# DreamOneX/yet-another-bpe

Measured on AMD Instinct MI355X. Metric: merges_per_sec, higher is better.
Workload: dtype u16

## Files before the change

include/yabpe.h:

```cpp
#ifndef YABPE_H
#define YABPE_H

#include <stddef.h>
#include <stdint.h>

#ifdef __cplusplus
extern "C" {
#endif

#define YABPE_ABI_VERSION 2

enum {
    YABPE_OK = 0,
    YABPE_E_INVALID = -1,
    YABPE_E_NODEVICE = -2,
    YABPE_E_HIP = -3,
    YABPE_E_CAPACITY = -4,
    YABPE_E_INTERNAL = -5,
    YABPE_E_COMM = -6,
    YABPE_E_UTF8 = -7
};

#define YABPE_LOAD_DEDUP 0x1u

// ... 44 lines not shown
    uint64_t table_entries;
    uint64_t retiles, table_rebuilds;
    double load_ms;
    double train_ms;
    double apply_ms_sampled;
    uint64_t apply_launches_sampled;
    uint64_t apply_algo_bytes_sampled;
    uint64_t apply_actual_bytes_sampled;
    uint64_t algo_bytes_total;
    double scan_ms_sampled;
    uint64_t scan_launches_sampled;
    uint64_t scan_algo_bytes_sampled;
    uint64_t scan_actual_bytes_sampled;
    uint64_t scan_skip_launches;
    uint64_t scan_skip_tiles_read;
    uint64_t cand_rebuilds;
    uint64_t cand_rescans;
    uint64_t fused_launches;
    double dense_ms_sampled;
    uint64_t dense_launches_sampled;
    uint64_t dense_algo_bytes_sampled;
    uint64_t dense_actual_bytes_sampled;
    double sparse_ms;
    uint64_t sparse_merges;
    double tail_ms;
    uint64_t tail_merges;
    uint64_t exchanges, exchange_bytes, exchange_cap_records, exchange_growths, exchange_max_records;
    uint64_t sparse_launches;
    uint64_t tail_launches;
    double exchange_ms_sampled;
    uint64_t exchanges_sampled;
    uint64_t exchange_p2p;
    uint64_t dense_launches, dense_merges;
} yabpe_stats_t;
int yabpe_stats(yabpe_ctx *ctx, yabpe_stats_t *out);
int yabpe_iter_log(yabpe_ctx *ctx, uint64_t *out_sites, uint64_t *out_live_slots, uint32_t cap, uint32_t *out_n);

int yabpe_event_log(yabpe_ctx *ctx, uint32_t *out_iter, float *out_us, float *out_scan_us, uint32_t cap, uint32_t *out_n);

typedef struct yabpe_latency_t {
    double launch_gap_us;
    double load_trip_us;
    double coherent_trip_us;
    double atomic_trip_us;
} yabpe_latency_t;
int yabpe_latency_probe(yabpe_ctx *ctx, yabpe_latency_t *out);

int yabpe_verify_table(yabpe_ctx *ctx, uint64_t *out_mismatches);
int yabpe_stream_checksum(yabpe_ctx *ctx, uint64_t *out_sum, uint64_t *out_words, uint64_t *out_tokens);

int yabpe_synth_generate(yabpe_ctx *ctx, uint64_t target_bytes, uint32_t n_types, uint64_t seed,
                         const uint8_t *alphabet, uint32_t alphabet_len, int space_prefix,
                         uint8_t **out_dev_bytes, uint64_t **out_dev_off, uint64_t *out_n_words, uint64_t *out_n_bytes);
int yabpe_synth_generate_lex(yabpe_ctx *ctx, uint64_t target_bytes, uint32_t n_types, uint64_t seed,
                             const uint8_t *lex_bytes, const uint64_t *lex_off,
                             uint8_t **out_dev_bytes, uint64_t **out_dev_off, uint64_t *out_n_pieces, uint64_t *out_n_bytes);
int yabpe_synth_free(yabpe_ctx *ctx);
int yabpe_memcpy_d2h(yabpe_ctx *ctx, void *dst_host, const void *src_dev, uint64_t n);
int yabpe_memcpy_h2d(yabpe_ctx *ctx, void *dst_dev, const void *src_host, uint64_t n);

int yabpe_pretokenize(yabpe_ctx *ctx, const uint8_t *text, uint64_t n_bytes, const uint64_t *chunk_off, uint32_t n_chunks,
                      const uint8_t *special_bytes, const uint32_t *special_off, uint32_t n_special,
                      const uint8_t **out_dev_text, uint64_t **out_dev_word_off, uint64_t *out_n_words, int64_t *out_bad_pos);
int yabpe_pretokenize_free(yabpe_ctx *ctx);

int yabpe_pool_add(yabpe_ctx *ctx, const uint8_t *bytes, const uint64_t *word_off, const uint64_t *word_freq, uint64_t n_words);
// ... 109 lines not shown
```

yet-another-bpe_amd/csrc/yabpe.hip:

```cpp
#include <hip/hip_runtime.h>
#include <dlfcn.h>
#include <rccl/rccl.h>

#include <algorithm>
#include <cstdarg>
#include <cstddef>
#include <cstdio>
#include <cstring>
#include <map>
#include <mutex>
#include <string>
#include <vector>

#include "../../include/yabpe.h"
#include "yabpe_kernels.h"
#include "yabpe_aux_kernels.h"
#include "yabpe_devmem.h"
#include "yabpe_pretok_kernels.h"
#include "yabpe_encode_kernels.h"
#include "yabpe_dropout_kernels.h"
#include "yabpe_decode_kernels.h"
#include "yabpe_layout_kernels.h"
#include "yabpe_replay_kernels.h"
#include "yabpe_pool_kernels.h"
// ... 19 lines not shown
        tried = true;
        std::vector<std::string> names;
        Dl_info info;
        if (dladdr((void *)&hipGetDeviceCount, &info) && info.dli_fname) {
            std::string dir(info.dli_fname);
            const size_t slash = dir.rfind('/');
            if (slash != std::string::npos) {
                dir.resize(slash);
                names.push_back(dir + "/librccl.so.1");
                names.push_back(dir + "/librccl.so");
            }
        }
        names.push_back("librccl.so.1");
        names.push_back("librccl.so");
        for (const auto &name : names) {
            r.h = dlopen(name.c_str(), RTLD_NOW | RTLD_LOCAL);
            if (r.h) break;
        }
        if (r.h) {
            r.GetUniqueId = (decltype(r.GetUniqueId))dlsym(r.h, "ncclGetUniqueId");
            r.CommInitRank = (decltype(r.CommInitRank))dlsym(r.h, "ncclCommInitRank");
            r.AllGather = (decltype(r.AllGather))dlsym(r.h, "ncclAllGather");
            r.AllReduce = (decltype(r.AllReduce))dlsym(r.h, "ncclAllReduce");
            r.CommDestroy = (decltype(r.CommDestroy))dlsym(r.h, "ncclCommDestroy");
            r.GetErrorString = (decltype(r.GetErrorString))dlsym(r.h, "ncclGetErrorString");
            if (!r.GetUniqueId || !r.CommInitRank || !r.AllGather || !r.AllReduce || !r.CommDestroy) r.h = nullptr;
        }
    }
    return r.h ? &r : nullptr;
}

constexpr uint32_t MAX_APPLY_BLOCKS = 8192;
constexpr uint32_t MAX_LISTS = 2048;
thread_local std::string g_create_error;

struct EventPair {
    hipEvent_t e0, e1, e2;
    uint32_t iter_rel;
    bool split;
};

}

struct yabpe_ctx {
    int device = 0;
    int n_cu = 256;
    int apply_occ = 4;
    hipStream_t stream = nullptr;
    std::string err;
    std::map<std::string, int64_t> opt;

    bool have_vocab = false;
    uint32_t base_tokens = 0;
    TokTable tt{};
    bool have_words = false;
    bool weighted = false;
    uint64_t n_words = 0, n_words_input = 0, tokens_initial = 0;
    uint32_t n_tiles = 0;
    uint16_t *tiles = nullptr, *tiles_alt = nullptr;
    uint32_t tiles_cap = 0, tiles_alt_cap = 0;
    uint32_t *tile_len = nullptr, *tile_len_alt = nullptr;
    uint32_t *tile_wbase = nullptr, *tile_wbase_alt = nullptr;
    uint32_t *wfreq = nullptr;
    uint32_t n_long = 0;
    uint16_t *long_tok = nullptr;
    unsigned long long *long_sig = nullptr;
// ... 31 lines not shown
    unsigned long long *enc_spans = nullptr;
    yabpe_encode_stats_t enc_stats{};
    unsigned long long enc_sums[4] = {0, 0, 0, 0};
    bool enc_done = false;
    hipEvent_t enc_ev[8] = {};
    bool have_dec_model = false;
    uint2 *dec_ent = nullptr;
    uint8_t *dec_pool = nullptr;
    uint32_t dec_n = 0;
    uint8_t *dec_text = nullptr;
    unsigned long long *dec_doc = nullptr;
    yabpe_decode_stats_t dec_stats{};
    hipEvent_t dec_ev[7] = {};
    uint32_t *lay_buf[3] = {};
    yabpe_layout_stats_t lay_stats{};
    hipEvent_t lay_ev[4] = {};
    yabpe_resume_stats_t resume_stats{};
    bool have_pool = false;
    PoolView wpool{};
    uint64_t wpool_arena_cap = 0, wpool_n = 0, wpool_bytes = 0;
    yabpe_pool_stats_t wpool_stats{};
    hipEvent_t wpool_ev[4] = {};
    unsigned long long *scratch64 = nullptr;
    unsigned long long *blk_stats = nullptr;
    uint32_t blk_used = 0;
    bool split_mode = false;
    uint32_t kmax_now = 1;
    uint32_t rec_n_live = 0;
    std::vector<float> ev_scan_us;
    unsigned long long *sig = nullptr;
    uint32_t sig_stride = 0;
    unsigned long long *blk_read = nullptr;
    uint64_t scan_skip_launches = 0;
    bool sig_valid = false;
    uint32_t sig_built_at = 0;
    uint64_t sig_tokens_at_build = 0;
    uint64_t sig_builds = 0;
    CandState *cand_state = nullptr;
    uint32_t cand_built_at = 0;
    unsigned long long cand_best_at_build = 0;
    uint32_t *sel_ticket = nullptr;
    unsigned long long *cand = nullptr;
    bool use_cand = false;
    uint64_t cand_rebuilds = 0, cand_rescans = 0;
    double cand_margin = 0.2;
    uint32_t cand_n_at_build = 0;
    bool pending = false;
    uint64_t fused_launches = 0;
    int rank = 0, n_ranks = 1;
    bool multi = false;
    ncclComm_t comm = nullptr;
    yabpe_allgather_fn ag_fn = nullptr;
    void *ag_user = nullptr;
    unsigned long long *xsmall = nullptr;
    uint8_t *xsend = nullptr, *xrecv = nullptr;
    uint64_t exchange_growths = 0;
    uint64_t exchange_max_records = 0;
    uint32_t xcap = 0;
    uint64_t xstride = 0;
    uint32_t xeff = 0;
    uint64_t xeff_sum = 0;
    uint32_t xseen[4] = {0, 0, 0, 0};
    uint64_t exchanges = 0;
    bool p2p = false;
    uint8_t *p2p_area = nullptr;
    std::vector<uint8_t *> p2p_peer;
// ... 1024 lines not shown
    c->stats.retiles = 0;
    c->stats.train_ms = 0;
    c->stats.apply_ms_sampled = 0;
    c->stats.apply_launches_sampled = 0;
    c->stats.apply_algo_bytes_sampled = 0;
    c->stats.apply_actual_bytes_sampled = 0;
    c->stats.dense_ms_sampled = 0;
    c->stats.dense_launches_sampled = 0;
    c->stats.dense_launches = 0;
    c->stats.dense_merges = 0;
    c->stats.dense_algo_bytes_sampled = 0;
    c->stats.dense_actual_bytes_sampled = 0;
    c->stats.sparse_ms = 0;
    c->stats.sparse_merges = 0;
    c->stats.sparse_launches = 0;
    c->stats.tail_ms = 0;
    c->stats.tail_merges = 0;
    c->stats.tail_launches = 0;
    c->stats.exchange_ms_sampled = 0;
    c->stats.exchanges_sampled = 0;
    c->stats.scan_ms_sampled = 0;
    c->stats.scan_launches_sampled = 0;
    c->stats.scan_algo_bytes_sampled = 0;
    c->stats.scan_actual_bytes_sampled = 0;
    c->scan_skip_launches = 0;
    c->cand_rebuilds = c->cand_rescans = 0;
    c->fused_launches = 0;
    c->exchanges = 0;
    c->xeff = c->xcap;
    c->xseen[0] = c->xseen[1] = c->xseen[2] = c->xseen[3] = 0;
    c->xeff_sum = 0;
    c->exchange_growths = 0;
    c->exchange_max_records = 0;
    if (c->blk_read) HIPCHK(c, hipMemsetAsync(c->blk_read, 0, MAX_LISTS * 8, c->stream));
    c->stats.algo_bytes_total = 0;
    c->have_words = true;
    return YABPE_OK;
}

int yabpe_load_words(yabpe_ctx *c, const uint8_t *bytes, const uint64_t *word_off, const uint64_t *word_freq,
                     uint64_t n_words, uint32_t flags) {
    if (!c) return YABPE_E_INVALID;
    return load_words_impl(c, bytes, word_off, word_freq, n_words, flags, nullptr);
}

int yabpe_load_words_resumed(yabpe_ctx *c, const uint8_t *bytes, const uint64_t *word_off, const uint64_t *word_freq, uint64_t n_words,
                             uint32_t flags, const uint32_t *merge_left, const uint32_t *merge_right, const uint32_t *merge_merged,
                             uint32_t n_merges) {
    if (!c) return YABPE_E_INVALID;
    HIPCHK(c, hipSetDevice(c->device));
    if (!c->have_vocab) return fail(c, YABPE_E_INVALID, "call yabpe_set_vocab first (with all of the model's tokens)");
    if (n_merges == 0) return load_words_impl(c, bytes, word_off, word_freq, n_words, flags, nullptr);
    if (!word_freq && !(flags & YABPE_LOAD_DEDUP))
        return fail(c, YABPE_E_INVALID, "a resumed load needs the pooled layout: pass word_freq or YABPE_LOAD_DEDUP");
    if (c->multi) return fail(c, YABPE_E_INVALID, "a resumed load on several GPUs is not supported");
    if (!merge_left || !merge_right || !merge_merged) return fail(c, YABPE_E_INVALID, "merge triples are NULL");
    TRY(state_pull(c));
    const uint32_t n_tokens = c->st_host->n_tokens;
    std::vector<uint32_t> len(n_tokens);
    HIPCHK(c, hipMemcpy(len.data(), c->tt.len, (size_t)n_tokens * 4, hipMemcpyDeviceToHost));
    for (uint32_t i = 0; i < n_merges; ++i) {
        const uint32_t l = merge_left[i], r = merge_right[i], m = merge_merged[i];
        if (l >= n_tokens || r >= n_tokens || m >= n_tokens)
            return fail(c, YABPE_E_INVALID, "merge %u names token id %u, the vocabulary has %u", i, std::max(l, std::max(r, m)), n_tokens);
        if (len[m] != len[l] + len[r])
            return fail(c, YABPE_E_INVALID, "merge %u: token %u has %u bytes, its operands %u + %u", i, m, len[m], len[l], len[r]);
    }
// ... 81 lines not shown
            F.ticket = c->sel_ticket;
            F.sel = select_params(c, rec_base, 0u, std::max(c->blk_used, grid_now));
        }
        return F;
    };
    if (c->n_tiles) {
        ApplyParams P{c->tiles, c->tile_len, c->tile_wbase, c->wfreq, c->n_tiles, out_table, c->st, c->blk_stats,
                      c->split_mode ? c->sig : nullptr, c->sig_stride, (uint32_t)AGG_N - 1u, 1u};
        if (!c->split_mode) {
            const FuseParams F = fuse_params(apply_grid);
            const uint32_t rr_blocks = rank_rides ? rank_blocks : 0u;
            c->blk_used = std::max(c->blk_used, apply_grid);
            if (c->weighted)
                hipLaunchKernelGGL(k_apply<true>, dim3(apply_grid + rr_blocks + long_blocks), dim3(BLOCK), 0, c->stream, P, apply_grid, R, F, LW, apply_grid + rr_blocks);
            else if (optv(c, "hist", 1) && tokens_upper <= (uint32_t)HIST_V)
                hipLaunchKernelGGL((k_apply<false, true>), dim3(apply_grid + rr_blocks + long_blocks), dim3(BLOCK), 0, c->stream, P, apply_grid, R, F, LW, apply_grid + rr_blocks);
            else
                hipLaunchKernelGGL(k_apply<false>, dim3(apply_grid + rr_blocks + long_blocks), dim3(BLOCK), 0, c->stream, P, apply_grid, R, F, LW, apply_grid + rr_blocks);
            if (ev) HIPCHK(c, hipEventRecord(ev->e1, c->stream));
        } else {
            if (!sparse) return fail(c, YABPE_E_INTERNAL, "sparse form without signatures");
            int64_t wpb_opt = optv(c, "full_wpb", 0);
            if (wpb_opt <= 0)
                wpb_opt = (c->st_host->best_count <= (unsigned long long)optv(c, "wide_sites_per_cu", 20) * c->n_cu && (c->n_tiles + 2047u) / 2048u <= c->n_cu) ? 16 : 8;
            const uint32_t nw = wpb_opt >= 16 ? 16u : 8u;
            const uint32_t nt = nw * 64u;
            const uint32_t target = (uint32_t)std::max<int64_t>(1, optv(c, "full_skip_blocks", (int64_t)c->n_cu * (16 / nw)));
            const uint32_t ktm = (uint32_t)scan_kt_max((int)nw);
            const uint32_t chunk = std::min<uint32_t>(nt * ktm, std::max<uint32_t>(64u, (uint32_t)(((uint64_t)(c->n_tiles + target - 1) / target + 63u) / 64u * 64u)));
            const uint32_t kt = (chunk + nt - 1) / nt;
            const uint32_t n_chunks = (c->n_tiles + chunk - 1) / chunk;
            const uint32_t scan_grid = std::max(1u, std::min<uint32_t>(std::min<uint32_t>(n_chunks, target), MAX_LISTS));
            if (!c->blk_read) {
                TRY(dmalloc(c, &c->blk_read, MAX_LISTS));
                HIPCHK(c, hipMemsetAsync(c->blk_read, 0, MAX_LISTS * 8, c->stream));
            }
            if (optv(c, "agg_small", 1) && !c->weighted && c->st_host->best_count * 4 < 48ull * std::max<uint32_t>(1u, c->n_cu * 3))
                P.agg_mask = (uint32_t)(c->kmax_now > 2 ? AGG_N : nw >= 16 ? AGG_N / 2 : AGG_N / 4) - 1u;
            const uint32_t rr_blocks = rank_rides ? rank_blocks : 0u;
            ScanSkipParams SQ{P, c->blk_read, scan_grid, kt, chunk, R, fuse_params(scan_grid), LW, scan_grid + rr_blocks};
            c->blk_used = std::max(c->blk_used, scan_grid);
            const uint32_t grid = scan_grid + rr_blocks + long_blocks;
#define YB_LAUNCH_SPARSE(NW_)                                                                                        \
    do {                                                                                                             \
        if (c->weighted)                                                                                             \
            hipLaunchKernelGGL((k_scan_skip<true, NW_>), dim3(grid), dim3(NW_ * 64), 0, c->stream, c->st, SQ);      \
        else                                                                                                         \
            hipLaunchKernelGGL((k_scan_skip<false, NW_>), dim3(grid), dim3(NW_ * 64), 0, c->stream, c->st, SQ);     \
    } while (0)
            if (nw == 16) YB_LAUNCH_SPARSE(16);
            else YB_LAUNCH_SPARSE(8);
#undef YB_LAUNCH_SPARSE
            c->scan_skip_launches++;
            if (ev) HIPCHK(c, hipEventRecord(ev->e1, c->stream));
        }
    } else if (ev) {
        HIPCHK(c, hipEventRecord(ev->e1, c->stream));
    }
    if (ev) HIPCHK(c, hipEventRecord(ev->e2, c->stream));
    if (!fuse_kernel && c->n_long) hipLaunchKernelGGL(k_apply_long, dim3(cdiv64(c->n_long, long_group)), dim3(BLOCK), 0, c->stream, LW);
    if (c->multi) {
        const uint64_t xbytes = 16 + (uint64_t)c->xeff * sizeof(DeltaRec);
        const uint8_t *recv = c->xrecv;
        uint64_t rstride = xbytes;
        if (c->p2p) {
            XchgParams X{};
            X.send = c->xsend;
            for (int r = 0; r < c->n_ranks; ++r) X.peer[r] = c->p2p_peer[r];
            X.flags_off = c->p2p_flags_off;
            X.half_bytes = c->p2p_half;
            X.stride = c->p2p_stride;
            X.seq = ++c->p2p_seq;
            X.rank = (uint32_t)c->rank;
// ... 458 lines not shown
    uint32_t off = 0, len = 0;
    HIPCHK(c, hipMemcpy(&off, c->tt.off + id, 4, hipMemcpyDeviceToHost));
    HIPCHK(c, hipMemcpy(&len, c->tt.len + id, 4, hipMemcpyDeviceToHost));
    *out_len = len;
    if (out && cap >= len && len) HIPCHK(c, hipMemcpy(out, c->tt.pool + off, len, hipMemcpyDeviceToHost));
    return YABPE_OK;
}

int yabpe_stats(yabpe_ctx *c, yabpe_stats_t *out) {
    if (!c || !out) return YABPE_E_INVALID;
    HIPCHK(c, hipSetDevice(c->device));
    TRY(state_pull(c));
    c->stats.n_words = c->n_words;
    c->stats.n_words_input = c->n_words_input;
    c->stats.n_long_words = c->n_long;
    c->stats.tokens_initial = c->tokens_initial;
    c->stats.tokens_now = c->st_host->tokens_now;
    c->stats.merges_done = c->st_host->iter;
    c->stats.n_tiles = c->n_tiles;
    c->stats.live_slots = c->st_host->live_slots;
    c->stats.table_capacity = c->table_cap;
    c->stats.table_entries = c->st_host->table_entries;
    c->stats.cand_rebuilds = c->cand_rebuilds;
    c->stats.cand_rescans = c->cand_rescans;
    c->stats.fused_launches = c->fused_launches;
    c->stats.exchanges = c->exchanges;
    c->stats.exchange_bytes = (c->multi && c->exchanges) ? (16 + (c->xeff_sum / c->exchanges) * sizeof(DeltaRec)) * (uint64_t)c->n_ranks : 0;
    c->stats.exchange_cap_records = c->xcap;
    c->stats.exchange_p2p = c->p2p ? 1 : 0;
    c->stats.exchange_growths = c->exchange_growths;
    c->stats.exchange_max_records = c->exchange_max_records;
    c->stats.scan_skip_launches = c->scan_skip_launches;
    c->stats.scan_skip_tiles_read = 0;
    if (c->blk_read) {
        std::vector<unsigned long long> br(MAX_LISTS);
        HIPCHK(c, hipMemcpy(br.data(), c->blk_read, MAX_LISTS * 8, hipMemcpyDeviceToHost));
        for (auto v : br) c->stats.scan_skip_tiles_read += v;
    }
    *out = c->stats;
    return YABPE_OK;
}

int yabpe_latency_probe(yabpe_ctx *c, yabpe_latency_t *out) {
    if (!c || !out) return YABPE_E_INVALID;
    HIPCHK(c, hipSetDevice(c->device));
    size_t free_b = 0, total_b = 0;
    (void)hipMemGetInfo(&free_b, &total_b);
    const uint32_t n = free_b > (8ull << 30) ? (1u << 29) : (1u << 27);
    uint32_t *next = nullptr, *sink = nullptr;
    unsigned long long *ticks = nullptr;
    struct Guard {
        uint32_t *&a, *&b;
        unsigned long long *&t;
        ~Guard() { dfree(a); dfree(b); dfree(t); }
    } guard{next, sink, ticks};
    TRY(dmalloc(c, &next, n));
    TRY(dmalloc(c, &sink, 1));
    TRY(dmalloc(c, &ticks, 1));
    double trip[3] = {0, 0, 0};
    const uint32_t hops = 1024;
    for (int mode = 0; mode < 3; ++mode) {
        hipLaunchKernelGGL(k_chain_init, dim3(n / 256), dim3(256), 0, c->stream, next, n, (uint32_t)mode);
        hipLaunchKernelGGL(k_chain_walk, dim3(1), dim3(1), 0, c->stream, next, hops, mode, ticks, sink);
        HIPCHK(c, hipGetLastError());
        unsigned long long t = 0;
        HIPCHK(c, hipMemcpyAsync(&t, ticks, 8, hipMemcpyDeviceToHost, c->stream));
        HIPCHK(c, hipStreamSynchronize(c->stream));
        trip[mode] = (double)t / 100.0 / hops;
    }
    hipEvent_t e0, e1;
// ... 91 lines not shown
        hipLaunchKernelGGL(k_long_checksum, dim3(cdiv64(c->n_long, BLOCK)), dim3(BLOCK), 0, c->stream, L);
        HIPCHK(c, hipGetLastError());
    }
    unsigned long long r[3];
    HIPCHK(c, hipMemcpyAsync(r, &c->scratch64[4], 24, hipMemcpyDeviceToHost, c->stream));
    HIPCHK(c, hipStreamSynchronize(c->stream));
    if (out_sum) *out_sum = r[0];
    if (out_words) *out_words = r[1];
    if (out_tokens) *out_tokens = r[2];
    return YABPE_OK;
}

int yabpe_memcpy_d2h(yabpe_ctx *c, void *dst_host, const void *src_dev, uint64_t n) {
    if (!c) return YABPE_E_INVALID;
    HIPCHK(c, hipSetDevice(c->device));
    HIPCHK(c, hipMemcpy(dst_host, src_dev, n, hipMemcpyDeviceToHost));
    return YABPE_OK;
}

#ifdef YB_PROFILE_SCAN
int yabpe_debug_sel_profile(unsigned long long out[16]) {
    return hipMemcpyFromSymbol(out, HIP_SYMBOL(yb::g_sel_prof), 128) == hipSuccess ? 0 : -1;
}
int yabpe_debug_sel_acc(unsigned long long out[72]) {
    return hipMemcpyFromSymbol(out, HIP_SYMBOL(yb::g_sel_acc), 72 * 8) == hipSuccess ? 0 : -1;
}
int yabpe_debug_ss_profile(unsigned long long out[8]) {
    return hipMemcpyFromSymbol(out, HIP_SYMBOL(yb::g_ss_prof), 64) == hipSuccess ? 0 : -1;
}
int yabpe_debug_launch_profile(unsigned long long *out, int reset) {
    if (reset) {
        std::vector<unsigned long long> z(65536 * 4, 0ull);
        for (size_t i = 0; i < 65536; ++i) z[i * 4] = ~0ull;
        return hipMemcpyToSymbol(HIP_SYMBOL(yb::g_launch_prof), z.data(), z.size() * 8) == hipSuccess ? 0 : -1;
    }
    return hipMemcpyFromSymbol(out, HIP_SYMBOL(yb::g_launch_prof), (size_t)65536 * 32) == hipSuccess ? 0 : -1;
}
int yabpe_debug_stop_hist(unsigned long long *out) {
    return hipMemcpyFromSymbol(out, HIP_SYMBOL(yb::g_stop_hist), (size_t)65536 * 8) == hipSuccess ? 0 : -1;
}
int yabpe_debug_scan_profile(unsigned long long *out, uint32_t n_blocks) {
    return hipMemcpyFromSymbol(out, HIP_SYMBOL(yb::g_scan_prof), (size_t)std::min<uint32_t>(n_blocks, yb::MAX_LISTS_PROF) * 64) == hipSuccess ? 0 : -1;
}
int yabpe_debug_flush_profile(unsigned long long *out, uint32_t n_blocks) {
    return hipMemcpyFromSymbol(out, HIP_SYMBOL(yb::g_flush_prof), (size_t)std::min<uint32_t>(n_blocks, yb::FLUSH_PROF_BLOCKS) * 32) == hipSuccess ? 0 : -1;
}
#endif
#ifdef YB_PROFILE_SLOW
int yabpe_debug_slow_profile(unsigned long long out[8]) {
    return hipMemcpyFromSymbol(out, HIP_SYMBOL(yb::g_slow_prof), 64) == hipSuccess ? 0 : -1;
}
#endif

int yabpe_memcpy_h2d(yabpe_ctx *c, void *dst_dev, const void *src_host, uint64_t n) {
    if (!c) return YABPE_E_INVALID;
    HIPCHK(c, hipSetDevice(c->device));
    HIPCHK(c, hipMemcpy(dst_dev, src_host, n, hipMemcpyHostToDevice));
    return YABPE_OK;
}

int yabpe_synth_generate(yabpe_ctx *c, uint64_t target_bytes, uint32_t n_types, uint64_t seed, const uint8_t *alphabet,
                         uint32_t alphabet_len, int space_prefix, uint8_t **out_dev_bytes, uint64_t **out_dev_off,
                         uint64_t *out_n_words, uint64_t *out_n_bytes) {
    if (!c || !alphabet || !alphabet_len || !n_types || !out_dev_bytes || !out_dev_off || !out_n_words || !out_n_bytes)
        return YABPE_E_INVALID;
    HIPCHK(c, hipSetDevice(c->device));
    SynthOut so{};
    int r = synth_generate(c->stream, target_bytes, n_types, seed, alphabet, alphabet_len, space_prefix, &so);
    if (r != 0) return fail(c, r == -2 ? YABPE_E_INTERNAL : YABPE_E_HIP, "synthetic generation failed (%d): %s", r, hipGetErrorString(hipGetLastError()));
    c->synth_bufs.push_back(so.bytes);
// ... 1090 lines not shown
```

yet-another-bpe_amd/csrc/yabpe_kernels.h:

```cpp
#pragma once
#include <hip/hip_runtime.h>
#include <stdint.h>

#include <type_traits>

#include "limit_logic.h"
#include "tile_logic.h"

namespace yb {

constexpr int CAP = 1024;
constexpr int LMAX = 64;
constexpr int SPAN = CAP - LMAX + 1;
constexpr int WPB = 4;
constexpr int BLOCK = WPB * 64;
constexpr int AGG_N = 1024;
constexpr uint32_t EMPTY = 0xFFFFFFFFu;
constexpr uint32_t PADPAD = (YB_PAD << 16) | YB_PAD;
constexpr int LONG_CH = 1024;
constexpr int SIG_ROWS = 512;
constexpr int SIG_ROWS_LOG2 = 9;
constexpr int SIG_TILES = 8;
constexpr int MAX_LISTS_PROF = 4096;
constexpr int SCAN_CHUNK = 256;
constexpr int SCAN_KT_MAX = 4;
constexpr int scan_kt_max(int nw) { return nw >= 16 ? 2 : 4; }

enum : uint32_t { HALT_NONE = 0, HALT_TABLE_FULL = 1, HALT_POOL_FULL = 2, HALT_VOCAB_FULL = 3, HALT_DELTA_FULL = 4, HALT_RESCAN = 5, HALT_COMM = 6 };

constexpr int KMAX = 16;
struct BatchMerge {
    uint32_t a, b, c, is_new;
};
struct DevState {
    uint32_t iter;
    uint32_t done;
    uint32_t halt;
    uint32_t halt_req;
    uint32_t a, b, c;
// ... 2506 lines not shown
            if (i + 1 < cnt) nxt = load_tile(P.tiles, tile + stride, __builtin_amdgcn_readlane(my_len, i + 1), lane);
            if (len == 0) continue;
            const uint32_t b0 = __builtin_amdgcn_readfirstlane(r.vb.x);
            const uint32_t na = next_lane(r.va.x, b0);
            const uint32_t nb = next_lane(r.vb.x, PADPAD);
            const uint32_t pmA = match_mask8(r.va, na, mk), pmB = match_mask8(r.vb, nb, mk);
            if (!__any((pmA | pmB) != 0u)) continue;
#ifdef YB_PROFILE_SLOW
            if (lane == 0 && t_end) W.prof[5] += __builtin_readcyclecounter() - t_end;
#endif
            {
                TileRegs rr = r;
                uint32_t len_io = len, fc = CAP;
                slow_tile<WEIGHTED, AggV, HIST, true>(C, W, tile, len_io, rr, na, nb, wave_sites, wave_freed, fc, pmA, pmB);
            }
#ifdef YB_PROFILE_SLOW
            t_end = __builtin_readcyclecounter();
#endif
        }
    }
#ifdef YB_PROFILE_SLOW
    if (lane < 8 && W.prof[lane]) atomicAdd(&g_slow_prof[lane], W.prof[lane]);
#endif
    apply_epilogue(P, C.agg, st, s_cnt, wave_sites, wave_freed, lane, HIST ? s_hist : nullptr, C.a, C.b, C.c);
    }
    __shared__ WinEnt s_selwin[WIN];
    fused_select_tail(F, s_selwin);
}

#ifdef YB_PROFILE_SCAN
#ifdef YB_PROFILE_LAUNCH
#define YB_LAUNCH_START(it) do { if (threadIdx.x == 0) atomicMin(&g_launch_prof[((it) & 0xFFFFu) * 4 + 0], wall_clock64()); } while (0)
#define YB_LAUNCH_END(it) do { if (threadIdx.x == 0) atomicMax(&g_launch_prof[((it) & 0xFFFFu) * 4 + 1], wall_clock64()); } while (0)
#else
#define YB_LAUNCH_START(it) do { } while (0)
#define YB_LAUNCH_END(it) do { } while (0)
#endif
__device__ unsigned long long g_scan_prof[MAX_LISTS_PROF * 8];
#define YB_SCAN_STAMP(i)                                                                       \
    do {                                                                                       \
        if (threadIdx.x == 0 && blockIdx.x < MAX_LISTS_PROF) g_scan_prof[blockIdx.x * 8 + (i)] = wall_clock64(); \
    } while (0)
#else
#define YB_SCAN_STAMP(i) do { } while (0)
#define YB_LAUNCH_START(it) do { } while (0)
#define YB_LAUNCH_END(it) do { } while (0)
#endif
struct ScanSkipParams {
    ApplyParams A;
    unsigned long long *blk_read;
    uint32_t scan_blocks;
    uint32_t kt;
    uint32_t chunk;
    RankParams R;
    FuseParams F;
    LongParams LW;
    uint32_t long_first;
};

template <bool WEIGHTED, int NW>
__device__ __forceinline__ bool scan_skip_block(DevState *st, const ScanSkipParams &Q) {
    using AggV = typename std::conditional<WEIGHTED, unsigned long long, int>::type;
    constexpr int NT = NW * 64;
    constexpr int KTM = scan_kt_max(NW);
    __shared__ uint32_t s_n, s_claim;
    __shared__ uint2 s_list[NT * KTM];
    __shared__ uint32_t s_keys[AGG_N];
    __shared__ AggV s_vals[AGG_N];
    __shared__ __attribute__((aligned(16))) WaveLds s_w[NW];
    __shared__ unsigned long long s_cnt[2];
    __shared__ BatchLds s_bm;
    const ApplyParams &P = Q.A;
    YB_SCAN_STAMP(0);
    const uint32_t st_stop = st->done | st->halt;
    const uint32_t nb_ = min(st->n_batch, (uint32_t)KMAX);
    const int lane = threadIdx.x & 63;
    const int wib = __builtin_amdgcn_readfirstlane(threadIdx.x >> 6);
    if (blockIdx.x < Q.scan_blocks && threadIdx.x < (uint32_t)KMAX) {
        const uint32_t k = threadIdx.x;
        BatchMerge m = BatchMerge{0u, 0u, 0u, 0u};
        if (k < nb_) m = st->batch[k];
        const SigHash H = sig_hash(yb_pairkey(m.a, m.b));
        s_bm.a[k] = m.a;
        s_bm.b[k] = m.b;
        s_bm.c[k] = m.c;
        s_bm.row[k] = H.row;
        s_bm.mask[k] = H.mask;
    }
    if (blockIdx.x < Q.scan_blocks) {
        agg_init(Agg<AggV>{s_keys, s_vals, P.agg_mask}, NT);
        wave_lds_init(s_w[wib], lane);
        if (threadIdx.x < 2) s_cnt[threadIdx.x] = 0;
        if (threadIdx.x == 0) {
            s_n = 0;
            s_claim = (uint32_t)NW;
        }
    }
    if (st_stop) return false;
    YB_SCAN_STAMP(5);
#ifdef YB_PROFILE_LAUNCH
    const uint32_t prof_it = st->iter;
    YB_LAUNCH_START(prof_it);
#endif
    if (blockIdx.x >= Q.scan_blocks) {
        if (NW > WPB && threadIdx.x >= BLOCK) return false;
        if (blockIdx.x >= Q.long_first)
            apply_long_block(Q.LW, blockIdx.x - Q.long_first);
        else
            rank_update_block(Q.R, blockIdx.x - Q.scan_blocks);
        YB_SCAN_STAMP(7);
        YB_LAUNCH_END(prof_it);
        return true;
    }
    const uint32_t n_blocks = Q.scan_blocks;
    const uint32_t nbatch = __builtin_amdgcn_readfirstlane(nb_);
    SlowCtx<AggV> C{P, Agg<AggV>{s_keys, s_vals, P.agg_mask}, st, 0u, 0u, 0u, 0u, 0u, lane,
                    KeyMemo{{EMPTY, EMPTY, EMPTY, EMPTY}, {0u, 0u, 0u, 0u}}};
    WaveLds &W = s_w[wib];
    __syncthreads();
    YB_SCAN_STAMP(6);
    uint32_t n_read = 0;
    unsigned long long wave_sites = 0, wave_freed = 0;
    const uint32_t kt = Q.kt;
    const uint32_t chunk = Q.chunk;
    const uint32_t n_chunks = (P.n_tiles + chunk - 1) / chunk;
    for (uint32_t ch = blockIdx.x; ch < n_chunks; ch += n_blocks) {
        uint32_t len[KTM], km[KTM];
        const uint32_t t_end = min(P.n_tiles, ch * chunk + chunk);
#pragma unroll
        for (uint32_t j = 0; j < (uint32_t)KTM; ++j) {
            const uint32_t t = ch * chunk + j * NT + threadIdx.x;
            len[j] = 0;
            km[j] = 0;
            if (j < kt && t < t_end) len[j] = P.tile_len[t];
        }
        constexpr uint32_t KG = KTM >= 4 ? 4u : 8u;
        for (uint32_t k0 = 0; k0 < nbatch; k0 += KG) {
            unsigned long long w[KG][KTM];
#pragma unroll
            for (uint32_t kk = 0; kk < KG; ++kk) {
                const bool on = k0 + kk < nbatch;
                const unsigned long long *rowp = P.sig + (size_t)s_bm.row[(k0 + kk) & (uint32_t)(KMAX - 1)] * P.sig_stride;
#pragma unroll
                for (uint32_t j = 0; j < (uint32_t)KTM; ++j) {
                    const uint32_t t = ch * chunk + j * NT + threadIdx.x;
                    w[kk][j] = (on && j < kt && t < t_end) ? rowp[t] : 0ull;
                }
            }
#pragma unroll
            for (uint32_t kk = 0; kk < KG; ++kk) {
                const unsigned long long mask = s_bm.mask[(k0 + kk) & (uint32_t)(KMAX - 1)];
                const bool on = k0 + kk < nbatch;
#pragma unroll
                for (uint32_t j = 0; j < (uint32_t)KTM; ++j)
                    if (on && (w[kk][j] & mask) == mask) km[j] |= 1u << (k0 + kk);
            }
        }
        YB_SCAN_STAMP(1);
#pragma unroll
        for (uint32_t j = 0; j < (uint32_t)KTM; ++j) {
            if (j >= kt) break;
            const bool mb = km[j] != 0 && len[j] != 0;
            const unsigned long long m = __ballot(mb);
            uint32_t base = 0;
            if (lane == 0 && m) base = atomicAdd(&s_n, (uint32_t)__popcll(m));
            base = __builtin_amdgcn_readfirstlane(base);
            if (mb) s_list[base + bits_below_lane(m)] = make_uint2(ch * chunk + j * NT + threadIdx.x, len[j] | (km[j] << 16));
        }
        __syncthreads();
        const uint32_t n = s_n;
        n_read += n;
        auto list_at = [&](uint32_t idx) -> uint2 {
            const uint2 v = s_list[idx];
            return make_uint2(__builtin_amdgcn_readfirstlane(v.x), __builtin_amdgcn_readfirstlane(v.y));
        };
        TileRegs pend = TileRegs{make_uint4(0u, 0u, 0u, 0u), make_uint4(0u, 0u, 0u, 0u)};
        uint32_t pend_tile = 0, pend_len = 0, pend_fc = CAP;
        auto write_back = [&](const TileRegs &t, uint32_t tile_, uint32_t len_, uint32_t fc_) {
            const uint32_t pad_end = (len_ + 7u) & ~7u;
            uint4 *wb = reinterpret_cast<uint4 *>(P.tiles + (size_t)tile_ * CAP);
            const uint32_t gA = (uint32_t)lane * 8u, gB = 512u + (uint32_t)lane * 8u;
            if (gA + 8u > fc_ && gA < pad_end) wb[lane] = t.va;
            if (gB + 8u > fc_ && gB < pad_end) wb[64 + lane] = t.vb;
            if (lane == 0) P.tile_len[tile_] = len_;
        };
        auto claim = [&]() -> uint32_t {
            uint32_t nx = 0;
            if (lane == 0) nx = atomicAdd(&s_claim, 1u);
            return __builtin_amdgcn_readfirstlane(nx);
        };
        uint32_t j = wib;
        uint32_t jn = j < n ? claim() : n;
        uint2 it0 = j < n ? list_at(j) : make_uint2(0u, 0u);
        TileRegs q0 = load_tile(P.tiles, it0.x, it0.y & 0xffffu, lane);
        while (j < n) {
            const uint32_t tile = it0.x;
            uint32_t tlen = it0.y & 0xffffu, kmask = it0.y >> 16;
            TileRegs r = q0;
            asm volatile("" : "+v"(r.va.x), "+v"(r.vb.x));
            if (pend_fc < (uint32_t)CAP) {
// ... 33 lines not shown
                        const unsigned long long t0 = __builtin_readcyclecounter();
                        vm_drain();
                        const unsigned long long t1 = __builtin_readcyclecounter();
                        if (lane == 0 && blockIdx.x == 7) {
                            atomicAdd(&g_ss_prof[5], t1 - t0);
                            atomicAdd(&g_ss_prof[6], 1ull);
                        }
                    }
#endif
                } else {
                    slow_tile<WEIGHTED, AggV, false, true, true>(C, W, tile, tlen, r, na, nb, wave_sites, wave_freed, first_changed, mine & 0xffu, mine >> 8);
                }
            }
            pend = r;
            pend_tile = tile;
            pend_len = tlen;
            pend_fc = first_changed;
            (void)len_in;
            if (j < n) jn = claim();
        }
        if (pend_fc < (uint32_t)CAP) write_back(pend, pend_tile, pend_len, pend_fc);
        __syncthreads();
        YB_SCAN_STAMP(2);
#ifdef YB_PROFILE_SCAN
        if (threadIdx.x == 0 && blockIdx.x < MAX_LISTS_PROF) g_scan_prof[blockIdx.x * 8 + 3] = ((unsigned long long)nbatch << 32) | n;
#endif
        if (threadIdx.x == 0) {
            uint32_t zero, first;
            asm volatile("v_mov_b32 %0, 0" : "=v"(zero));
            asm volatile("v_mov_b32 %0, %1" : "=v"(first) : "n"(NW));
            s_n = zero;
            s_claim = first;
        }
        __syncthreads();
    }
    if (threadIdx.x == 0 && Q.blk_read) Q.blk_read[blockIdx.x] += n_read;
    YB_SCAN_STAMP(4);
    apply_epilogue<AggV, NT>(P, C.agg, st, s_cnt, wave_sites, wave_freed, lane);
    YB_SCAN_STAMP(7);
    YB_LAUNCH_END(prof_it);
    return true;
}
template <bool WEIGHTED, int NW>
__global__ __launch_bounds__(NW * 64, 16 / NW) void k_scan_skip(DevState *st, ScanSkipParams Q) {
    __shared__ WinEnt s_selwin[WIN];
    if (!scan_skip_block<WEIGHTED, NW>(st, Q)) return;
    fused_select_tail(Q.F, s_selwin);
}

struct RehashParams {
    PairTable from, to;
    DevState *st;
};
__global__ __launch_bounds__(BLOCK) void k_rehash(RehashParams P) {
    const uint32_t cap = P.from.cap;
    for (uint32_t s = blockIdx.x * BLOCK + threadIdx.x; s < cap; s += gridDim.x * BLOCK) {
        const uint32_t k = P.from.keys[s];
        if (k == EMPTY) continue;
        const long long v = (long long)P.from.cnt[s];
        if (v != 0) gt_add(P.to, P.st, k, v);
    }
}


struct DeltaApplyParams {
    const uint8_t *recv;
    uint32_t n_ranks, cap;
    unsigned long long stride;
    PairTable table;
    DevState *st;
    FuseParams F;
    uint32_t peer_written;
// ... 197 lines not shown
```

yet-another-bpe_amd/yet_another_bpe/_native.py:

```python
from __future__ import annotations

import ctypes
import os
from ctypes import POINTER, byref, c_char_p, c_double, c_int, c_int64, c_uint8, c_uint32, c_uint64, c_void_p
from pathlib import Path

import numpy as np

_CSRC = Path(__file__).resolve().parent.parent / "csrc"
LIB_PATH = Path(os.environ.get("YABPE_LIB", _CSRC / "libyabpe.so"))


class YabpeError(RuntimeError):
    def __init__(self, code: int, msg: str):
        super().__init__(f"yabpe error {code}: {msg}")
        self.code = code


class Utf8Error(ValueError):

    def __init__(self, position: int):
        super().__init__(f"invalid UTF-8 at byte {position}")
        self.position = position


E_CAPACITY = -4
E_UTF8 = -7


class Stats(ctypes.Structure):
    _fields_ = [(n, c_uint64) for n in (
        "n_words", "n_words_input", "n_long_words", "tokens_initial", "tokens_now", "merges_done", "n_tiles",
        "live_slots", "table_capacity", "table_entries", "retiles", "table_rebuilds")] + [
        ("load_ms", c_double), ("train_ms", c_double), ("apply_ms_sampled", c_double)] + [(n, c_uint64) for n in (
            "apply_launches_sampled", "apply_algo_bytes_sampled", "apply_actual_bytes_sampled", "algo_bytes_total")] + [
        ("scan_ms_sampled", c_double)] + [(n, c_uint64) for n in (
            "scan_launches_sampled", "scan_algo_bytes_sampled", "scan_actual_bytes_sampled", "scan_skip_launches", "scan_skip_tiles_read", "cand_rebuilds", "cand_rescans", "fused_launches")] + [
        ("dense_ms_sampled", c_double)] + [(n, c_uint64) for n in ("dense_launches_sampled", "dense_algo_bytes_sampled", "dense_actual_bytes_sampled")] + [
        ("sparse_ms", c_double), ("sparse_merges", c_uint64), ("tail_ms", c_double), ("tail_merges", c_uint64)] + [
        (n, c_uint64) for n in ("exchanges", "exchange_bytes", "exchange_cap_records", "exchange_growths", "exchange_max_records", "sparse_launches", "tail_launches")] + [("exchange_ms_sampled", c_double), ("exchanges_sampled", c_uint64), ("exchange_p2p", c_uint64),
        ("dense_launches", c_uint64), ("dense_merges", c_uint64)]


class EncodeStats(ctypes.Structure):
    _fields_ = [(n, c_uint64) for n in ("n_bytes", "n_docs", "n_pretokens", "n_unique", "n_unique_long", "n_specials", "n_ids")] + [
        (n, c_double) for n in ("split_ms", "pretok_ms", "pool_ms", "words_ms", "emit_ms", "total_ms")]


class DecodeStats(ctypes.Structure):
    _fields_ = [(n, c_uint64) for n in ("n_ids", "n_docs", "n_unknown", "n_gathered", "n_bytes", "n_replacements", "n_docs_repaired")] + [
        (n, c_double) for n in ("lengths_ms", "gather_ms", "check_ms", "repair_ms", "total_ms")]


class LayoutStats(ctypes.Structure):
    _fields_ = [(n, c_uint64) for n in ("n_ids", "n_docs", "n_rows", "row_len", "n_truncated_docs", "n_ids_dropped", "n_pad_slots")] + [
        (n, c_double) for n in ("lengths_ms", "write_ms", "total_ms")]


class Layout(ctypes.Structure):
    _fields_ = [(n, c_uint32) for n in ("row_len", "pad_id", "bos_id", "eos_id", "flags")]


class ResumeStats(ctypes.Structure):
    _fields_ = [(n, c_uint64) for n in ("n_unique", "n_long", "tokens")] + [(n, c_double) for n in ("segment_ms", "build_ms")]


class PoolStats(ctypes.Structure):
    _fields_ = [(n, c_uint64) for n in ("n_calls", "n_words_added", "n_empty_dropped", "n_unique", "n_bytes", "slot_capacity",
                                        "arena_capacity", "slot_growths", "arena_growths")] + [
        (n, c_double) for n in ("pool_ms", "probe_ms", "append_ms", "total_ms")]


class Latency(ctypes.Structure):
    _fields_ = [(n, c_double) for n in ("launch_gap_us", "load_trip_us", "coherent_trip_us", "atomic_trip_us")]
# ... 590 lines not shown
```

Baseline: 46980.

## Add dynamic work-stealing of leftover scan tiles in sparse scan-skip kernel

In the sparse scan-skip kernel with 8 waves per block, each block first processes its static chunk. The remaining tiles are then split into smaller pieces that blocks claim dynamically through a tagged global atomic counter, instead of following a fixed round-robin stride over chunks. The aim is to reduce load imbalance and tail latency when tiles outnumber scan_grid*chunk. This adds one atomic claim plus a block barrier per piece and a per-block pieces-taken counter, and it adds profiling instrumentation and a stat field.

Measured after the change: 48190, median of 6. 1.03x the previous value.

```diff
diff --git a/include/yabpe.h b/include/yabpe.h
--- a/include/yabpe.h
+++ b/include/yabpe.h
@@ -100,6 +100,7 @@
     uint64_t exchanges_sampled;
     uint64_t exchange_p2p;
     uint64_t dense_launches, dense_merges;
+    uint64_t scan_skip_pieces_taken;
 } yabpe_stats_t;
 int yabpe_stats(yabpe_ctx *ctx, yabpe_stats_t *out);
 int yabpe_iter_log(yabpe_ctx *ctx, uint64_t *out_sites, uint64_t *out_live_slots, uint32_t cap, uint32_t *out_n);
diff --git a/yet-another-bpe_amd/csrc/steal_logic.h b/yet-another-bpe_amd/csrc/steal_logic.h
--- /dev/null
+++ b/yet-another-bpe_amd/csrc/steal_logic.h
@@ -0,0 +1,31 @@
+#pragma once
+#include <stdint.h>
+
+#include "tile_logic.h"
+
+#define YB_STEAL_TAG_SHIFT 24
+#define YB_STEAL_IDX_MASK ((1ull << YB_STEAL_TAG_SHIFT) - 1ull)
+
+YB_HD unsigned long long yb_steal_arm(unsigned long long tag) { return tag << YB_STEAL_TAG_SHIFT; }
+YB_HD bool yb_steal_current(unsigned long long word, unsigned long long tag) { return (word >> YB_STEAL_TAG_SHIFT) == tag; }
+YB_HD uint32_t yb_steal_idx(unsigned long long word) { return (uint32_t)(word & YB_STEAL_IDX_MASK); }
+
+template <class Ops>
+YB_HD uint32_t yb_steal_claim(Ops &ops, unsigned long long tag) {
+    unsigned long long old = ops.add(1ull);
+    if (!yb_steal_current(old, tag)) {
+        ops.max(yb_steal_arm(tag));
+        old = ops.add(1ull);
+    }
+    return yb_steal_idx(old);
+}
+
+YB_HD uint32_t yb_piece_tiles(uint32_t rest, uint32_t blocks, uint32_t chunk) {
+    if (blocks == 0u) blocks = 1u;
+    unsigned long long p = ((unsigned long long)rest + blocks - 1u) / blocks;
+    p = (p + 63ull) / 64ull * 64ull;
+    if (p < 256ull) p = 256ull;
+    if (p > (unsigned long long)chunk) p = chunk;
+    return (uint32_t)p;
+}
+YB_HD uint32_t yb_piece_count(uint32_t rest, uint32_t piece) { return piece ? (uint32_t)(((unsigned long long)rest + piece - 1u) / piece) : 0u; }
diff --git a/yet-another-bpe_amd/csrc/yabpe.hip b/yet-another-bpe_amd/csrc/yabpe.hip
--- a/yet-another-bpe_amd/csrc/yabpe.hip
+++ b/yet-another-bpe_amd/csrc/yabpe.hip
@@ -75,6 +75,7 @@
 
 constexpr uint32_t MAX_APPLY_BLOCKS = 8192;
 constexpr uint32_t MAX_LISTS = 2048;
+constexpr uint32_t BLK_READ_WORDS = 2 * MAX_LISTS + 16;
 thread_local std::string g_create_error;
 
 struct EventPair {
@@ -172,6 +173,7 @@
     uint32_t sig_stride = 0;
     unsigned long long *blk_read = nullptr;
     uint64_t scan_skip_launches = 0;
+    uint64_t piece_tag = 0;
     bool sig_valid = false;
     uint32_t sig_built_at = 0;
     uint64_t sig_tokens_at_build = 0;
@@ -1262,7 +1264,7 @@
     c->xeff_sum = 0;
     c->exchange_growths = 0;
     c->exchange_max_records = 0;
-    if (c->blk_read) HIPCHK(c, hipMemsetAsync(c->blk_read, 0, MAX_LISTS * 8, c->stream));
+    if (c->blk_read) HIPCHK(c, hipMemsetAsync(c->blk_read, 0, 2 * MAX_LISTS * 8, c->stream));
     c->stats.algo_bytes_total = 0;
     c->have_words = true;
     return YABPE_OK;
@@ -1410,13 +1412,18 @@
             const uint32_t n_chunks = (c->n_tiles + chunk - 1) / chunk;
             const uint32_t scan_grid = std::max(1u, std::min<uint32_t>(std::min<uint32_t>(n_chunks, target), MAX_LISTS));
             if (!c->blk_read) {
-                TRY(dmalloc(c, &c->blk_read, MAX_LISTS));
-                HIPCHK(c, hipMemsetAsync(c->blk_read, 0, MAX_LISTS * 8, c->stream));
+                TRY(dmalloc(c, &c->blk_read, BLK_READ_WORDS));
+                HIPCHK(c, hipMemsetAsync(c->blk_read, 0, BLK_READ_WORDS * 8, c->stream));
             }
+            const uint32_t rest = c->n_tiles - std::min<uint64_t>(c->n_tiles, (uint64_t)scan_grid * chunk);
+            const bool pieces = rest && nw == 8 && optv(c, "chunk_steal", 1);
+            const uint32_t piece = !rest ? 0u : pieces ? yb_piece_tiles(rest, scan_grid, chunk) : chunk;
             if (optv(c, "agg_small", 1) && !c->weighted && c->st_host->best_count * 4 < 48ull * std::max<uint32_t>(1u, c->n_cu * 3))
                 P.agg_mask = (uint32_t)(c->kmax_now > 2 ? AGG_N : nw >= 16 ? AGG_N / 2 : AGG_N / 4) - 1u;
             const uint32_t rr_blocks = rank_rides ? rank_blocks : 0u;
-            ScanSkipParams SQ{P, c->blk_read, scan_grid, kt, chunk, R, fuse_params(scan_grid), LW, scan_grid + rr_blocks};
+            ScanSkipParams SQ{P, c->blk_read, scan_grid, kt, chunk, R, fuse_params(scan_grid), LW, scan_grid + rr_blocks,
+                              piece, pieces ? yb_piece_count(rest, piece) : 0u, pieces ? c->blk_read + 2 * MAX_LISTS : nullptr,
+                              pieces ? ++c->piece_tag : 0ull, c->blk_read + MAX_LISTS};
             c->blk_used = std::max(c->blk_used, scan_grid);
             const uint32_t grid = scan_grid + rr_blocks + long_blocks;
 #define YB_LAUNCH_SPARSE(NW_)                                                                                        \
@@ -1941,10 +1948,12 @@
     c->stats.exchange_max_records = c->exchange_max_records;
     c->stats.scan_skip_launches = c->scan_skip_launches;
     c->stats.scan_skip_tiles_read = 0;
+    c->stats.scan_skip_pieces_taken = 0;
     if (c->blk_read) {
-        std::vector<unsigned long long> br(MAX_LISTS);
-        HIPCHK(c, hipMemcpy(br.data(), c->blk_read, MAX_LISTS * 8, hipMemcpyDeviceToHost));
-        for (auto v : br) c->stats.scan_skip_tiles_read += v;
+        std::vector<unsigned long long> br(2 * MAX_LISTS);
+        HIPCHK(c, hipMemcpy(br.data(), c->blk_read, 2 * MAX_LISTS * 8, hipMemcpyDeviceToHost));
+        for (uint32_t i = 0; i < MAX_LISTS; ++i) c->stats.scan_skip_tiles_read += br[i];
+        for (uint32_t i = MAX_LISTS; i < 2 * MAX_LISTS; ++i) c->stats.scan_skip_pieces_taken += br[i];
     }
     *out = c->stats;
     return YABPE_OK;
@@ -2102,10 +2111,21 @@
     if (reset) {
         std::vector<unsigned long long> z(65536 * 4, 0ull);
         for (size_t i = 0; i < 65536; ++i) z[i * 4] = ~0ull;
+#ifdef YB_PROFILE_LAUNCH
+        {
+            std::vector<unsigned long long> zw(65536 * 8, 0ull);
+            if (hipMemcpyToSymbol(HIP_SYMBOL(yb::g_launch_wg), zw.data(), zw.size() * 8) != hipSuccess) return -1;
+        }
+#endif
         return hipMemcpyToSymbol(HIP_SYMBOL(yb::g_launch_prof), z.data(), z.size() * 8) == hipSuccess ? 0 : -1;
     }
     return hipMemcpyFromSymbol(out, HIP_SYMBOL(yb::g_launch_prof), (size_t)65536 * 32) == hipSuccess ? 0 : -1;
 }
+#ifdef YB_PROFILE_LAUNCH
+int yabpe_debug_launch_wg(unsigned long long *out) {
+    return hipMemcpyFromSymbol(out, HIP_SYMBOL(yb::g_launch_wg), (size_t)65536 * 64) == hipSuccess ? 0 : -1;
+}
+#endif
 int yabpe_debug_stop_hist(unsigned long long *out) {
     return hipMemcpyFromSymbol(out, HIP_SYMBOL(yb::g_stop_hist), (size_t)65536 * 8) == hipSuccess ? 0 : -1;
 }
diff --git a/yet-another-bpe_amd/csrc/yabpe_kernels.h b/yet-another-bpe_amd/csrc/yabpe_kernels.h
--- a/yet-another-bpe_amd/csrc/yabpe_kernels.h
+++ b/yet-another-bpe_amd/csrc/yabpe_kernels.h
@@ -5,6 +5,7 @@
 #include <type_traits>
 
 #include "limit_logic.h"
+#include "steal_logic.h"
 #include "tile_logic.h"
 
 namespace yb {
@@ -2577,6 +2578,21 @@
 #ifdef YB_PROFILE_LAUNCH
 #define YB_LAUNCH_START(it) do { if (threadIdx.x == 0) atomicMin(&g_launch_prof[((it) & 0xFFFFu) * 4 + 0], wall_clock64()); } while (0)
 #define YB_LAUNCH_END(it) do { if (threadIdx.x == 0) atomicMax(&g_launch_prof[((it) & 0xFFFFu) * 4 + 1], wall_clock64()); } while (0)
+__device__ unsigned long long g_launch_wg[65536 * 8];
+#define YB_LAUNCH_WG_END(it, ncand, t_cand)                                             \
+    do {                                                                                \
+        if (threadIdx.x == 0) {                                                         \
+            unsigned long long *w_ = &g_launch_wg[((it) & 0xFFFFu) * 8];                \
+            const unsigned long long e_ = wall_clock64();                               \
+            atomicAdd(&w_[0], e_);                                                      \
+            atomicAdd(&w_[1], 1ull);                                                    \
+            atomicMax(&w_[2], e_);                                                      \
+            atomicAdd(&w_[3], (unsigned long long)(ncand));                             \
+            atomicMax(&w_[4], (unsigned long long)(ncand));                             \
+            atomicAdd(&w_[5], (unsigned long long)(t_cand));                            \
+            atomicMax(&w_[6], (unsigned long long)(t_cand));                            \
+        }                                                                               \
+    } while (0)
 #else
 #define YB_LAUNCH_START(it) do { } while (0)
 #define YB_LAUNCH_END(it) do { } while (0)
@@ -2601,6 +2617,16 @@
     FuseParams F;
     LongParams LW;
     uint32_t long_first;
+    uint32_t piece;
+    uint32_t n_pieces;
+    unsigned long long *piece_ctr;
+    unsigned long long piece_tag;
+    unsigned long long *piece_taken;
+};
+struct PieceCtrOps {
+    unsigned long long *p;
+    __device__ __forceinline__ unsigned long long add(unsigned long long v) { return atomicAdd(p, v); }
+    __device__ __forceinline__ void max(unsigned long long v) { atomicMax(p, v); }
 };
 
 template <bool WEIGHTED, int NW>
@@ -2608,7 +2634,9 @@
     using AggV = typename std::conditional<WEIGHTED, unsigned long long, int>::type;
     constexpr int NT = NW * 64;
     constexpr int KTM = scan_kt_max(NW);
+    constexpr bool DYN = NW == 8;
     __shared__ uint32_t s_n, s_claim;
+    __shared__ uint32_t s_piece;
     __shared__ uint2 s_list[NT * KTM];
     __shared__ uint32_t s_keys[AGG_N];
     __shared__ AggV s_vals[AGG_N];
@@ -2668,13 +2696,13 @@
     unsigned long long wave_sites = 0, wave_freed = 0;
     const uint32_t kt = Q.kt;
     const uint32_t chunk = Q.chunk;
-    const uint32_t n_chunks = (P.n_tiles + chunk - 1) / chunk;
-    for (uint32_t ch = blockIdx.x; ch < n_chunks; ch += n_blocks) {
+    uint32_t t0 = blockIdx.x * chunk;
+    while (t0 < P.n_tiles) {
         uint32_t len[KTM], km[KTM];
-        const uint32_t t_end = min(P.n_tiles, ch * chunk + chunk);
+        const uint32_t t_end = min(P.n_tiles, t0 + ((DYN && Q.piece_ctr && t0 >= n_blocks * chunk) ? Q.piece : chunk));
 #pragma unroll
         for (uint32_t j = 0; j < (uint32_t)KTM; ++j) {
-            const uint32_t t = ch * chunk + j * NT + threadIdx.x;
+            const uint32_t t = t0 + j * NT + threadIdx.x;
             len[j] = 0;
             km[j] = 0;
             if (j < kt && t < t_end) len[j] = P.tile_len[t];
@@ -2688,7 +2716,7 @@
                 const unsigned long long *rowp = P.sig + (size_t)s_bm.row[(k0 + kk) & (uint32_t)(KMAX - 1)] * P.sig_stride;
 #pragma unroll
                 for (uint32_t j = 0; j < (uint32_t)KTM; ++j) {
-                    const uint32_t t = ch * chunk + j * NT + threadIdx.x;
+                    const uint32_t t = t0 + j * NT + threadIdx.x;
                     w[kk][j] = (on && j < kt && t < t_end) ? rowp[t] : 0ull;
                 }
             }
@@ -2710,7 +2738,7 @@
             uint32_t base = 0;
             if (lane == 0 && m) base = atomicAdd(&s_n, (uint32_t)__popcll(m));
             base = __builtin_amdgcn_readfirstlane(base);
-            if (mb) s_list[base + bits_below_lane(m)] = make_uint2(ch * chunk + j * NT + threadIdx.x, len[j] | (km[j] << 16));
+            if (mb) s_list[base + bits_below_lane(m)] = make_uint2(t0 + j * NT + threadIdx.x, len[j] | (km[j] << 16));
         }
         __syncthreads();
         const uint32_t n = s_n;
@@ -2810,12 +2838,36 @@
             s_n = zero;
             s_claim = first;
         }
+        const uint32_t piece = Q.piece;
+        const bool more = piece != 0u;
+        if (DYN && more && Q.piece_ctr && threadIdx.x == 0) {
+            PieceCtrOps ops{Q.piece_ctr};
+            const uint32_t pc = yb_steal_claim(ops, Q.piece_tag);
+            s_piece = pc;
+            if (pc < Q.n_pieces) Q.piece_taken[blockIdx.x] += 1ull;
+        }
         __syncthreads();
+        if (!more) break;
+        const uint32_t rest0 = n_blocks * chunk;
+        if (DYN && Q.piece_ctr) {
+            const uint32_t pc = __builtin_amdgcn_readfirstlane(s_piece);
+            if (pc >= Q.n_pieces) break;
+            t0 = rest0 + pc * piece;
+        } else {
+            if (t0 + rest0 < t0) break;
+            t0 += rest0;
+        }
     }
     if (threadIdx.x == 0 && Q.blk_read) Q.blk_read[blockIdx.x] += n_read;
     YB_SCAN_STAMP(4);
+#ifdef YB_PROFILE_LAUNCH
+    const unsigned long long prof_tc = wall_clock64();
+#endif
     apply_epilogue<AggV, NT>(P, C.agg, st, s_cnt, wave_sites, wave_freed, lane);
     YB_SCAN_STAMP(7);
+#ifdef YB_PROFILE_LAUNCH
+    YB_LAUNCH_WG_END(prof_it, n_read, prof_tc);
+#endif
     YB_LAUNCH_END(prof_it);
     return true;
 }
diff --git a/yet-another-bpe_amd/yet_another_bpe/_native.py b/yet-another-bpe_amd/yet_another_bpe/_native.py
--- a/yet-another-bpe_amd/yet_another_bpe/_native.py
+++ b/yet-another-bpe_amd/yet_another_bpe/_native.py
@@ -39,7 +39,7 @@
         ("dense_ms_sampled", c_double)] + [(n, c_uint64) for n in ("dense_launches_sampled", "dense_algo_bytes_sampled", "dense_actual_bytes_sampled")] + [
         ("sparse_ms", c_double), ("sparse_merges", c_uint64), ("tail_ms", c_double), ("tail_merges", c_uint64)] + [
         (n, c_uint64) for n in ("exchanges", "exchange_bytes", "exchange_cap_records", "exchange_growths", "exchange_max_records", "sparse_launches", "tail_launches")] + [("exchange_ms_sampled", c_double), ("exchanges_sampled", c_uint64), ("exchange_p2p", c_uint64),
-        ("dense_launches", c_uint64), ("dense_merges", c_uint64)]
+        ("dense_launches", c_uint64), ("dense_merges", c_uint64), ("scan_skip_pieces_taken", c_uint64)]
 
 
 class EncodeStats(ctypes.Structure):
```
